# dcharatan/pixelsplat

Hardware: NVIDIA H100
Metric: rendered views/sec fwd+bwd @256x256, 3 gauss/px (higher is better)
Workload: dtype f32

## Files before the change

### include/pixelsplat_b200.h

```cpp
#ifndef PIXELSPLAT_B200_H
#define PIXELSPLAT_B200_H

#include <stddef.h>
#include <stdint.h>

#ifdef __cplusplus
extern "C" {
#endif

#if defined(__GNUC__)
#define PS_API __attribute__((visibility("default")))
#else
#define PS_API
#endif

#define PS_OK 0
#define PS_ERR_INVALID_ARGUMENT 1
#define PS_ERR_CUDA 2
#define PS_ERR_UNSUPPORTED 3

#define PS_TILE 16

#define PS_SH_M3 0
#define PS_SH_3M 1
// ... 21 lines not shown
#define PS_DEPTH_NONE 0
#define PS_DEPTH_Z 1
#define PS_DEPTH_DISPARITY 2
#define PS_DEPTH_RELATIVE_DISPARITY 3
#define PS_DEPTH_LOG 4

typedef struct ps_raster_inputs {
    const float *means;
    const float *cov;
    const float *opacities;
    const float *sh;
    const float *viewmatrix;
    const float *projmatrix;
    const float *campos;
    const float *tanfov;
    const float *background;
    const float *scene_scale;
    const float *near_far;
} ps_raster_inputs;

typedef struct ps_raster_state {
    void *geom;    size_t geom_bytes;
    void *binning; size_t binning_bytes;
    void *image;   size_t image_bytes;
} ps_raster_state;

typedef struct ps_raster_sizes {
    size_t geom_bytes, binning_bytes, image_bytes, backward_bytes;
} ps_raster_sizes;

typedef struct ps_raster_layout {
    size_t depth;
    size_t radii;
    size_t xy;
    size_t conic_opacity;
    size_t rgb;
    size_t rect;
    size_t clamped;
    size_t tile_count;
    size_t tile_start;
    size_t tile_cursor;
    size_t n_instances;
    size_t vis_pairs;
    size_t vis_any;
    size_t keys;
    size_t keys_alt;
    size_t final_T;
    size_t n_contrib;
    size_t cull;
    size_t color;
    size_t block_hits;
    size_t run_hits;
    size_t run_state;
    size_t depth_image;
    size_t run_depth;
} ps_raster_layout;

typedef struct ps_raster_camera_grads {
    float *d_viewmatrix;
    float *d_projmatrix;
    float *d_campos;
    float *d_tanfov;
    void *workspace;
    size_t workspace_bytes;
} ps_raster_camera_grads;

typedef struct ps_raster_grads {
    float *d_means;
    float *d_cov;
    float *d_opacities;
    float *d_sh;
    float *d_means2d;
    const ps_raster_camera_grads *camera;
} ps_raster_grads;

PS_API int ps_raster_camera_workspace_bytes(const ps_raster_desc *desc, size_t *out);

PS_API int ps_version(void);
PS_API const char *ps_last_error(void);

PS_API unsigned long long ps_launch_count(void);
PS_API void ps_timing_enable(int on);
PS_API int ps_timing_read(float *ms);

PS_API int ps_set_option(const char *name, int value);
PS_API int ps_get_option(const char *name, int *value);

PS_API int ps_raster_sizes_query(const ps_raster_desc *desc, ps_raster_sizes *out);
PS_API int ps_raster_layout_query(const ps_raster_desc *desc, ps_raster_layout *out);

PS_API int ps_camera_setup(int32_t n_views, const float *extrinsics, const float *intrinsics,
                           const float *near_plane, const float *far_plane, int32_t scale_invariant,
                           float *viewmatrix, float *projmatrix, float *campos, float *tanfov,
                           float *scene_scale, void *stream);

PS_API int ps_camera_setup_backward(int32_t n_views, const float *extrinsics, const float *intrinsics,
                                    const float *near_plane, const float *far_plane, int32_t scale_invariant,
                                    const float *d_viewmatrix, const float *d_projmatrix, const float *d_campos,
                                    const float *d_tanfov, float *d_extrinsics, float *d_intrinsics, void *stream);

PS_API int ps_raster_forward(const ps_raster_desc *desc, const ps_raster_inputs *in,
                      const ps_raster_state *state, float *out_color, int32_t *out_radii,
                      int64_t *n_instances_host, void *stream);

PS_API int ps_raster_backward(const ps_raster_desc *desc, const ps_raster_inputs *in,
                       const ps_raster_state *state, const float *d_color ,
                       void *scratch, size_t scratch_bytes, const ps_raster_grads *grads,
                       void *stream);


PS_API int ps_raster_backward_depth(const ps_raster_desc *desc, const ps_raster_inputs *in,
                                    const ps_raster_state *state, const float *d_color ,
                                    const float *loss_target, const float *grad_scale, const float *d_depth,
                                    void *scratch, size_t scratch_bytes, const ps_raster_grads *grads,
                                    void *stream);

#define PS_LOSS_SLOTS 64
typedef struct ps_raster_loss {
    const float *target;
    float *sums;
} ps_raster_loss;

PS_API int ps_raster_forward_loss(const ps_raster_desc *desc, const ps_raster_inputs *in,
                                  const ps_raster_state *state, const ps_raster_loss *loss,
                                  float *out_color , int32_t *out_radii,
                                  int64_t *n_instances_host, void *stream);
PS_API int ps_raster_backward_loss(const ps_raster_desc *desc, const ps_raster_inputs *in,
                                   const ps_raster_state *state, const float *target ,
                                   const float *grad_scale ,
                                   void *scratch, size_t scratch_bytes, const ps_raster_grads *grads,
                                   void *stream);

typedef struct ps_epipolar_desc {
    int32_t batch, views;
    int32_t grid_h, grid_w;
    int32_t samples;
    int32_t channels;
    int32_t heads;
    int32_t pe_dim;
} ps_epipolar_desc;

typedef struct ps_epipolar_inputs {
    const float *features;
    const float *segments;
    const uint8_t *valid;
    const float *rel_disparity;
    const float *q_feat;
    const float *q_pe;
    const float *bias;
} ps_epipolar_inputs;

PS_API int ps_epipolar_geometry(int32_t batch, int32_t views, int32_t grid_h, int32_t grid_w,
                                int32_t samples, const float *extrinsics ,
                                const float *intrinsics , const float *near_plane,
                                const float *far_plane , float *segments, uint8_t *valid,
                                float *rel_disparity, float *t_range, void *stream);

PS_API int ps_epipolar_attention_forward(const ps_epipolar_desc *desc, const ps_epipolar_inputs *in,
                                         float *z, float *e, float *mass, float *lse, void *stream);

PS_API int ps_epipolar_attention_backward(const ps_epipolar_desc *desc, const ps_epipolar_inputs *in,
                                          const float *lse, const float *dz, const float *de,
                                          const float *dmass, const float *d_row, float *dq_feat,
                                          float *dq_pe, float *dbias, float *dfeatures, void *stream);

PS_API int ps_epipolar_attention_backward_workspace_bytes(const ps_epipolar_desc *desc, size_t *out);
// ... 163 lines not shown
```

### pixelsplat_b200/_lib.py

```python
from __future__ import annotations

import ctypes
import os
from pathlib import Path

_PKG = Path(__file__).resolve().parent
LIB_PATH = Path(os.environ.get("PIXELSPLAT_B200_LIB", _PKG / "_C" / "libpixelsplat_b200.so"))

PS_OK = 0
PS_SH_M3, PS_SH_3M = 0, 1
PS_COV_TRIU6, PS_COV_3X3 = 0, 1
PS_SH_BASIS_3DGS, PS_SH_BASIS_E3NN = 0, 1
PS_ERR_UNSUPPORTED = 3
DEPTH_MODES = {None: 0, "depth": 1, "disparity": 2, "relative_disparity": 3, "log": 4}
TILE = 16

_ERR_NAMES = {1: "PS_ERR_INVALID_ARGUMENT", 2: "PS_ERR_CUDA", 3: "PS_ERR_UNSUPPORTED"}


class RasterDesc(ctypes.Structure):
    _fields_ = [
        ("n_scenes", ctypes.c_int32), ("views_per_scene", ctypes.c_int32),
        ("n_gaussians", ctypes.c_int32), ("sh_coeffs", ctypes.c_int32),
        ("sh_degree", ctypes.c_int32), ("sh_layout", ctypes.c_int32),
# ... 43 lines not shown
                ("sh_coeffs", ctypes.c_int32), ("image_h", ctypes.c_int32), ("image_w", ctypes.c_int32),
                ("scale_min", ctypes.c_float), ("scale_max", ctypes.c_float), ("eps", ctypes.c_float),
                ("reserved", ctypes.c_int32)]


class AdapterInputs(ctypes.Structure):
    _fields_ = [(n, ctypes.c_void_p) for n in (
        "extrinsics", "intrinsics", "sh_rotation", "sh_mask", "coordinates", "depths", "raw")]


class RasterLoss(ctypes.Structure):
    _fields_ = [("target", ctypes.c_void_p), ("sums", ctypes.c_void_p)]


LOSS_SLOTS = 64
LPIPS_MAX_LAYERS = 5


class LpipsLayer(ctypes.Structure):
    _fields_ = [("x0", ctypes.c_void_p), ("x1", ctypes.c_void_p), ("weight", ctypes.c_void_p),
                ("C", ctypes.c_int32), ("H", ctypes.c_int32), ("W", ctypes.c_int32)]


class LpipsDesc(ctypes.Structure):
    _fields_ = [("n_layers", ctypes.c_int32), ("N", ctypes.c_int32), ("layers", LpipsLayer * LPIPS_MAX_LAYERS),
                ("dropout_seed", ctypes.c_void_p)]


class LpipsGrads(ctypes.Structure):
    _fields_ = [("d_x0", ctypes.c_void_p * LPIPS_MAX_LAYERS), ("d_x1", ctypes.c_void_p * LPIPS_MAX_LAYERS)]


class ResampleDesc(ctypes.Structure):
    _fields_ = [(n, ctypes.c_int32) for n in ("n_images", "in_h", "in_w", "out_h", "out_w", "taps_h", "taps_v")] + \
        [(n, ctypes.c_void_p) for n in ("images", "flip", "bounds_h", "weights_h", "bounds_v", "weights_v")]


PS_EVAL_RENDER, PS_EVAL_FRAME = 0, 1
EVAL_MAX_IMAGES = 32


class EvalDesc(ctypes.Structure):
    _fields_ = [(n, ctypes.c_int32) for n in ("mode", "n_images", "height", "width")] + \
        [(n, ctypes.c_void_p) for n in ("render", "frame_in", "target", "frame_out", "planes", "sse")]


CLIP_ADAM_CHUNK = 4096
CLIP_ADAM_SEGMENT_FIELDS = ("param", "grad", "exp_avg", "exp_avg_sq", "count", "first_chunk")


class ClipAdamDesc(ctypes.Structure):
    _fields_ = [("n_segments", ctypes.c_int32), ("reserved", ctypes.c_int32), ("n_chunks", ctypes.c_int64),
                ("warm_up_steps", ctypes.c_int64)] + \
        [(n, ctypes.c_double) for n in ("lr", "beta1", "beta2", "eps", "max_norm")]


class ClipAdamState(ctypes.Structure):
    _fields_ = [("step", ctypes.c_void_p), ("grad_norm", ctypes.c_void_p)]


class RasterCameraGrads(ctypes.Structure):
    _fields_ = [(n, ctypes.c_void_p) for n in ("d_viewmatrix", "d_projmatrix", "d_campos", "d_tanfov", "workspace")] + \
        [("workspace_bytes", ctypes.c_size_t)]


class RasterGrads(ctypes.Structure):
    _fields_ = [(n, ctypes.c_void_p) for n in (
        "d_means", "d_cov", "d_opacities", "d_sh", "d_means2d")] + [("camera", ctypes.POINTER(RasterCameraGrads))]


EXPORTS = ("ps_version", "ps_last_error", "ps_raster_sizes_query", "ps_raster_layout_query",
           "ps_raster_forward", "ps_raster_backward", "ps_camera_setup", "ps_launch_count",
           "ps_timing_enable", "ps_timing_read", "ps_epipolar_geometry",
           "ps_epipolar_attention_forward", "ps_epipolar_attention_backward",
           "ps_self_attention_forward", "ps_gaussian_adapter_forward", "ps_gaussian_adapter_backward",
           "ps_sh_rotation_matrices", "ps_set_option", "ps_raster_forward_loss", "ps_raster_backward_loss",
           "ps_self_attention_forward_stats", "ps_self_attention_backward", "ps_get_option",
           "ps_raster_backward_depth", "ps_ssim_workspace_bytes", "ps_ssim_forward", "ps_ssim_backward",
           "ps_epipolar_attention_backward_workspace_bytes", "ps_epipolar_attention_backward_deterministic",
           "ps_raster_camera_workspace_bytes", "ps_camera_setup_backward", "ps_lpips_workspace_bytes",
           "ps_lpips_forward", "ps_lpips_backward", "ps_vit_attention_forward",
           "ps_vit_attention_backward_workspace_bytes", "ps_vit_attention_backward", "ps_image_resample",
           "ps_eval_images_workspace_bytes", "ps_eval_images", "ps_clip_adam_segment_chunks",
           "ps_clip_adam_workspace_bytes", "ps_clip_adam_step")


class NativeLibraryMissing(ImportError):
    pass


def _load() -> ctypes.CDLL:
    if not LIB_PATH.exists():
        raise NativeLibraryMissing(
            f"{LIB_PATH} not found: the sm_90a CUDA library is not built. Run "
            f"`make -C {_PKG / 'csrc'}` (or __graft_entry__.build()). There is no CPU fallback.")
    lib = ctypes.CDLL(str(LIB_PATH))
    lib.ps_version.restype = ctypes.c_int
    lib.ps_last_error.restype = ctypes.c_char_p
    P = ctypes.POINTER
    lib.ps_raster_sizes_query.argtypes = [P(RasterDesc), P(RasterSizes)]
    lib.ps_raster_layout_query.argtypes = [P(RasterDesc), P(RasterLayout)]
    lib.ps_raster_forward.argtypes = [P(RasterDesc), P(RasterInputs), P(RasterState), ctypes.c_void_p,
                                      ctypes.c_void_p, ctypes.c_void_p, ctypes.c_void_p]
    lib.ps_raster_backward.argtypes = [P(RasterDesc), P(RasterInputs), P(RasterState), ctypes.c_void_p,
                                       ctypes.c_void_p, ctypes.c_size_t, P(RasterGrads), ctypes.c_void_p]
    lib.ps_raster_forward_loss.argtypes = [P(RasterDesc), P(RasterInputs), P(RasterState), P(RasterLoss),
                                           ctypes.c_void_p, ctypes.c_void_p, ctypes.c_void_p, ctypes.c_void_p]
    lib.ps_raster_backward_loss.argtypes = [P(RasterDesc), P(RasterInputs), P(RasterState), ctypes.c_void_p,
                                            ctypes.c_void_p, ctypes.c_void_p, ctypes.c_size_t, P(RasterGrads),
                                            ctypes.c_void_p]
    lib.ps_raster_backward_depth.argtypes = [P(RasterDesc), P(RasterInputs), P(RasterState)] + [ctypes.c_void_p] * 5 + \
        [ctypes.c_size_t, P(RasterGrads), ctypes.c_void_p]
    lib.ps_raster_backward_depth.restype = ctypes.c_int
    lib.ps_raster_forward_loss.restype = ctypes.c_int
    lib.ps_raster_backward_loss.restype = ctypes.c_int
    lib.ps_camera_setup.argtypes = [ctypes.c_int32] + [ctypes.c_void_p] * 4 + [ctypes.c_int32] + \
        [ctypes.c_void_p] * 6
    lib.ps_camera_setup.restype = ctypes.c_int
    lib.ps_camera_setup_backward.argtypes = [ctypes.c_int32] + [ctypes.c_void_p] * 4 + [ctypes.c_int32] + \
        [ctypes.c_void_p] * 7
    lib.ps_camera_setup_backward.restype = ctypes.c_int
    lib.ps_raster_camera_workspace_bytes.argtypes = [P(RasterDesc), P(ctypes.c_size_t)]
    lib.ps_raster_camera_workspace_bytes.restype = ctypes.c_int
    lib.ps_launch_count.restype = ctypes.c_ulonglong
    lib.ps_timing_enable.argtypes = [ctypes.c_int]
    lib.ps_timing_enable.restype = None
    lib.ps_timing_read.argtypes = [ctypes.POINTER(ctypes.c_float)]
    lib.ps_timing_read.restype = ctypes.c_int
    lib.ps_epipolar_geometry.argtypes = [ctypes.c_int32] * 5 + [ctypes.c_void_p] * 9
    lib.ps_epipolar_geometry.restype = ctypes.c_int
    lib.ps_epipolar_attention_forward.argtypes = [P(EpipolarDesc), P(EpipolarInputs)] + [ctypes.c_void_p] * 5
    lib.ps_epipolar_attention_forward.restype = ctypes.c_int
    lib.ps_epipolar_attention_backward.argtypes = [P(EpipolarDesc), P(EpipolarInputs)] + [ctypes.c_void_p] * 10
    lib.ps_epipolar_attention_backward.restype = ctypes.c_int
    lib.ps_epipolar_attention_backward_workspace_bytes.argtypes = [P(EpipolarDesc), P(ctypes.c_size_t)]
    lib.ps_epipolar_attention_backward_workspace_bytes.restype = ctypes.c_int
    lib.ps_epipolar_attention_backward_deterministic.argtypes = [P(EpipolarDesc), P(EpipolarInputs)] + \
        [ctypes.c_void_p] * 10 + [ctypes.c_size_t, ctypes.c_void_p]
    lib.ps_epipolar_attention_backward_deterministic.restype = ctypes.c_int
    lib.ps_self_attention_forward.argtypes = [ctypes.c_int32] * 4 + [ctypes.c_void_p, ctypes.c_float, ctypes.c_void_p,
                                                                      ctypes.c_int32, ctypes.c_void_p]
    lib.ps_self_attention_forward.restype = ctypes.c_int
    lib.ps_self_attention_forward_stats.argtypes = [ctypes.c_int32] * 4 + [ctypes.c_void_p, ctypes.c_float,
                                                                            ctypes.c_void_p, ctypes.c_void_p, ctypes.c_void_p]
    lib.ps_self_attention_forward_stats.restype = ctypes.c_int
    lib.ps_self_attention_backward.argtypes = [ctypes.c_int32] * 4 + [ctypes.c_void_p] * 4 + [ctypes.c_float,
                                                                                             ctypes.c_void_p, ctypes.c_void_p]
    lib.ps_self_attention_backward.restype = ctypes.c_int
    lib.ps_gaussian_adapter_forward.argtypes = [P(AdapterDesc), P(AdapterInputs)] + [ctypes.c_void_p] * 6
    lib.ps_gaussian_adapter_forward.restype = ctypes.c_int
    lib.ps_gaussian_adapter_backward.argtypes = [P(AdapterDesc), P(AdapterInputs)] + [ctypes.c_void_p] * 9
    lib.ps_gaussian_adapter_backward.restype = ctypes.c_int
    lib.ps_sh_rotation_matrices.argtypes = [ctypes.c_int32] * 4 + [ctypes.c_void_p] * 5
    lib.ps_sh_rotation_matrices.restype = ctypes.c_int
    lib.ps_set_option.argtypes = [ctypes.c_char_p, ctypes.c_int]
    lib.ps_set_option.restype = ctypes.c_int
    lib.ps_get_option.argtypes = [ctypes.c_char_p, ctypes.POINTER(ctypes.c_int)]
    lib.ps_get_option.restype = ctypes.c_int
    lib.ps_ssim_workspace_bytes.argtypes = [ctypes.c_int32] * 3 + [P(ctypes.c_size_t)]
    lib.ps_ssim_workspace_bytes.restype = ctypes.c_int
    lib.ps_ssim_forward.argtypes = [ctypes.c_int32] * 3 + [ctypes.c_void_p] * 4 + [ctypes.c_size_t, ctypes.c_void_p]
    lib.ps_ssim_forward.restype = ctypes.c_int
    lib.ps_ssim_backward.argtypes = [ctypes.c_int32] * 3 + [ctypes.c_void_p] * 6 + [ctypes.c_size_t, ctypes.c_void_p]
    lib.ps_ssim_backward.restype = ctypes.c_int
    lib.ps_lpips_workspace_bytes.argtypes = [P(LpipsDesc), P(ctypes.c_size_t)]
    lib.ps_lpips_workspace_bytes.restype = ctypes.c_int
    lib.ps_lpips_forward.argtypes = [P(LpipsDesc), ctypes.c_void_p, ctypes.c_void_p, ctypes.c_size_t, ctypes.c_void_p]
    lib.ps_lpips_forward.restype = ctypes.c_int
    lib.ps_lpips_backward.argtypes = [P(LpipsDesc), ctypes.c_void_p, P(LpipsGrads), ctypes.c_void_p]
    lib.ps_lpips_backward.restype = ctypes.c_int
    lib.ps_vit_attention_forward.argtypes = [ctypes.c_int32] * 4 + [ctypes.c_void_p, ctypes.c_float] + \
        [ctypes.c_void_p] * 3
    lib.ps_vit_attention_forward.restype = ctypes.c_int
    lib.ps_vit_attention_backward_workspace_bytes.argtypes = [ctypes.c_int32] * 4 + [P(ctypes.c_size_t)]
    lib.ps_vit_attention_backward_workspace_bytes.restype = ctypes.c_int
    lib.ps_vit_attention_backward.argtypes = [ctypes.c_int32] * 4 + [ctypes.c_void_p] * 4 + \
        [ctypes.c_float, ctypes.c_void_p, ctypes.c_void_p, ctypes.c_size_t, ctypes.c_void_p]
    lib.ps_vit_attention_backward.restype = ctypes.c_int
    lib.ps_image_resample.argtypes = [P(ResampleDesc), ctypes.c_void_p, ctypes.c_void_p]
    lib.ps_image_resample.restype = ctypes.c_int
    lib.ps_eval_images_workspace_bytes.argtypes = [ctypes.c_int32] * 3 + [P(ctypes.c_size_t)]
    lib.ps_eval_images_workspace_bytes.restype = ctypes.c_int
    lib.ps_eval_images.argtypes = [P(EvalDesc), ctypes.c_void_p, ctypes.c_size_t, ctypes.c_void_p]
    lib.ps_eval_images.restype = ctypes.c_int
    lib.ps_clip_adam_segment_chunks.argtypes = [ctypes.c_void_p, ctypes.c_int64]
    lib.ps_clip_adam_segment_chunks.restype = ctypes.c_int64
    lib.ps_clip_adam_workspace_bytes.argtypes = [P(ClipAdamDesc), P(ctypes.c_size_t)]
    lib.ps_clip_adam_workspace_bytes.restype = ctypes.c_int
    lib.ps_clip_adam_step.argtypes = [P(ClipAdamDesc), ctypes.c_void_p, P(ClipAdamState), ctypes.c_void_p,
                                      ctypes.c_size_t, ctypes.c_void_p]
    lib.ps_clip_adam_step.restype = ctypes.c_int
    for f in ("ps_raster_sizes_query", "ps_raster_layout_query", "ps_raster_forward", "ps_raster_backward"):
        getattr(lib, f).restype = ctypes.c_int
    return lib


lib = _load()


class NativeError(RuntimeError):
    pass


def check(rc: int, what: str) -> None:
    if rc != PS_OK:
        msg = lib.ps_last_error().decode("utf-8", "replace")
        exc = ValueError if rc == 1 else NativeError
        raise exc(f"{what}: {_ERR_NAMES.get(rc, rc)}: {msg}")


def on_device(device, fn, *args) -> int:
# ... 40 lines not shown
```

### pixelsplat_b200/csrc/ps_common.cuh

```cuda
#pragma once
#include <cuda_runtime.h>
#include <stdint.h>

#include "../../include/pixelsplat_b200.h"

namespace ps {

constexpr int kTile = PS_TILE;
constexpr int kTilePixels = kTile * kTile;

struct Geom {
    float *depth;
    int32_t *radii;
    float2 *xy;
    float4 *conic_opacity;
    float4 *rgb;
    ushort4 *rect;
    uint8_t *clamped;
    uint32_t *tile_count;
    uint32_t *tile_start;
    uint32_t *tile_cursor;
    long long *n_instances;
    uint32_t *vis_pairs;
    float4 *cull;
// ... 51 lines not shown
__device__ __forceinline__ float depth_value(int mode, float vz, const float *scale, const float *near_far, int vid) {
    const float z = scale ? vz / scale[vid] : vz;
    if (mode == PS_DEPTH_DISPARITY) return 1.0f / z;
    if (mode == PS_DEPTH_RELATIVE_DISPARITY) {
        const float dn = 1.0f / (near_far[2 * vid] + kDepthEps), df = 1.0f / (near_far[2 * vid + 1] + kDepthEps);
        return 1.0f - (1.0f / (z + kDepthEps) - df) / (dn - df + kDepthEps);
    }
    if (mode == PS_DEPTH_LOG) return logf(fmaxf(fminf(z, near_far[2 * vid]), near_far[2 * vid + 1]));
    return z;
}

__device__ __forceinline__ float depth_value_grad(int mode, float vz, const float *scale, const float *near_far, int vid) {
    const float z = scale ? vz / scale[vid] : vz;
    if (mode == PS_DEPTH_DISPARITY) return -1.0f / (z * z);
    if (mode == PS_DEPTH_RELATIVE_DISPARITY) {
        const float dn = 1.0f / (near_far[2 * vid] + kDepthEps), df = 1.0f / (near_far[2 * vid + 1] + kDepthEps);
        const float iz = 1.0f / (z + kDepthEps);
        return iz * iz / (dn - df + kDepthEps);
    }
    if (mode == PS_DEPTH_LOG) {
        const float nr = near_far[2 * vid], fr = near_far[2 * vid + 1];
        const float m = fminf(z, nr);
        const float gm = z < nr ? 1.0f : (z == nr ? 0.5f : 0.0f);
        const float gr = m > fr ? 1.0f : (m == fr ? 0.5f : 0.0f);
        return gm * gr / fmaxf(m, fr);
    }
    return 1.0f;
}

__device__ __forceinline__ float2 cull_extent(float a, float c, float o) {
    if (!(a > 0.0f) || !(c > 0.0f) || !(o <= 3.0e38f)) return make_float2(3.0e38f, 3.0e38f);
    if (!(o * 255.0f >= 1.0f - 1e-3f)) return make_float2(-3.0e38f, -3.0e38f);
    const float tau2 = 2.0f * (__logf(fmaxf(o * 255.0f, 1.0f)) + 0.01f);
    return make_float2(sqrtf(tau2 * a) * 1.001f + 0.01f, sqrtf(tau2 * c) * 1.001f + 0.01f);
}

constexpr uint32_t kLivePosLimit = 1u << 24;

__device__ __forceinline__ uint32_t tile_block_mask(const float4 &cr, int x0, int y0) {
    const float xl = cr.x - cr.z, xh = cr.x + cr.z, yl = cr.y - cr.w, yh = cr.y + cr.w;
    uint32_t xm = 0, m = 0;
#pragma unroll
    for (int bx = 0; bx < 2; ++bx)
        xm |= ((xh >= (float)(x0 + 8 * bx)) && (xl <= (float)(x0 + 8 * bx + 7))) ? 1u << bx : 0u;
#pragma unroll
    for (int by = 0; by < 4; ++by)
        m |= ((yh >= (float)(y0 + 4 * by)) && (yl <= (float)(y0 + 4 * by + 3))) ? xm << (2 * by) : 0u;
    return m;
}

void set_error(const char *fmt, ...);

enum Mark { kMarkFwdStart = 0, kMarkPreprocess, kMarkScatter, kMarkSort, kMarkCompositeFwd,
            kMarkBwdStart, kMarkBwdZero, kMarkCompositeBwd, kMarkPreprocessBwd, kNumMarks };
void mark(int id, cudaStream_t st);
void count_launch();

bool first_use_on_device(unsigned long long &mask);

#define PS_CUDA_CHECK(expr)                                                              \
    do {                                                                                 \
        cudaError_t _e = (expr);                                                         \
        if (_e != cudaSuccess) {                                                         \
            ps::set_error("%s failed: %s (%s:%d)", #expr, cudaGetErrorString(_e), __FILE__, __LINE__); \
            return PS_ERR_CUDA;                                                          \
        }                                                                                \
    } while (0)

#define PS_LAUNCH_CHECK(name)                                                            \
    do {                                                                                 \
        cudaError_t _e = cudaGetLastError();                                             \
        if (_e != cudaSuccess) {                                                         \
            ps::set_error("launch of %s failed: %s", name, cudaGetErrorString(_e));      \
            return PS_ERR_CUDA;                                                          \
        }                                                                                \
        ps::count_launch();                                                              \
    } while (0)

int launch_preprocess(const Dims &d, const Inputs &in, const Geom &g, cudaStream_t st);
int launch_sh_color(const Dims &d, const Inputs &in, const Geom &g, cudaStream_t st);
int launch_binning(const Dims &d, const Geom &g, unsigned long long *keys,
                   unsigned long long *keys_alt, int sort_impl, int segment_hint, cudaEvent_t scanned,
                   cudaStream_t st);
int launch_composite_forward(const Dims &d, const Inputs &in, const Geom &g,
                             const unsigned long long *keys, const uint2 *live, const ImageState &img,
                             float *out_color, const LossEpilogue &loss, const HitLists &hl, float *loss_partials,
                             cudaStream_t st);
int launch_composite_backward(const Dims &d, const Inputs &in, const Geom &g,
                              const unsigned long long *keys, const uint2 *live, const ImageState &img,
                              const float *d_color, const float *d_depth, const ViewGrads &vg,
                              const ViewGrads *records, const LossEpilogue &loss, const HitLists &hl,
                              cudaStream_t st);
int launch_composite_forward_v1(const Dims &d, const Inputs &in, const Geom &g,
                                const unsigned long long *keys, const ImageState &img,
                                float *out_color, cudaStream_t st);
int launch_composite_backward_v1(const Dims &d, const Inputs &in, const Geom &g,
                                 const unsigned long long *keys, const ImageState &img,
                                 const float *d_color, const ViewGrads &vg, cudaStream_t st);
int composite_impl();
int set_composite_option(int which, int value);
int get_composite_option(int which);
int composite_segments(long long tasks);
bool composite_hit_lists(long long capacity);
int launch_preprocess_backward(const Dims &d, const Inputs &in, const Geom &g, const ViewGrads &vg,
                               const ps_raster_grads &grads, cudaStream_t st);
int launch_clear_pair_grads(const Dims &d, const Geom &g, const ViewGrads &vg, cudaStream_t st);

}
```

### pixelsplat_b200/csrc/raster_api.cu

```cuda
#include <cstdarg>
#include <atomic>
#include <cstdio>
#include <cstring>
#include <mutex>

#include "ps_common.cuh"

namespace ps {

static thread_local char g_error[512] = "";

void set_error(const char *fmt, ...) {
    va_list ap;
    va_start(ap, fmt);
    vsnprintf(g_error, sizeof(g_error), fmt, ap);
    va_end(ap);
}

static bool g_timing = false;
static cudaEvent_t g_events[kNumMarks];
static bool g_events_ready = false;
static std::atomic<unsigned long long> g_launches{0};

void count_launch() { g_launches.fetch_add(1, std::memory_order_relaxed); }
// ... 183 lines not shown
}

static ImageState make_image(const Layout &L, void *image) {
    char *b = static_cast<char *>(image);
    ImageState im;
    im.final_T = reinterpret_cast<float *>(b + L.off.final_T);
    im.n_contrib = reinterpret_cast<uint32_t *>(b + L.off.n_contrib);
    im.color = reinterpret_cast<float *>(b + L.off.color);
    im.run_state = reinterpret_cast<float4 *>(b + L.off.run_state);
    im.depth_image = L.off.depth_image ? reinterpret_cast<float *>(b + L.off.depth_image) : nullptr;
    im.run_depth = L.off.run_depth ? reinterpret_cast<float *>(b + L.off.run_depth) : nullptr;
    return im;
}

static int check_common(const ps_raster_desc *desc, const ps_raster_inputs *in, const ps_raster_state *state,
                        const Layout &L, bool backward) {
    const size_t image_bytes = backward && L.det ? L.loss_partials : L.sizes.image_bytes;
    if (!in || !state) { set_error("inputs/state is NULL"); return PS_ERR_INVALID_ARGUMENT; }
    if (!in->means || !in->cov || !in->opacities || !in->sh || !in->viewmatrix || !in->projmatrix ||
        !in->campos || !in->tanfov || !in->background) {
        set_error("a required input pointer is NULL");
        return PS_ERR_INVALID_ARGUMENT;
    }
    if (!state->geom || !state->binning || !state->image) { set_error("a state buffer is NULL"); return PS_ERR_INVALID_ARGUMENT; }
    if (state->geom_bytes < L.sizes.geom_bytes || state->binning_bytes < L.sizes.binning_bytes ||
        state->image_bytes < image_bytes) {
        set_error("state buffers too small: need geom %zu binning %zu image %zu, got %zu %zu %zu",
                  L.sizes.geom_bytes, L.sizes.binning_bytes, image_bytes, state->geom_bytes,
                  state->binning_bytes, state->image_bytes);
        return PS_ERR_INVALID_ARGUMENT;
    }
    if (((uintptr_t)state->geom | (uintptr_t)state->binning | (uintptr_t)state->image) & 15) {
        set_error("state buffers must be 16-byte aligned");
        return PS_ERR_INVALID_ARGUMENT;
    }
    if ((desc->depth_mode == PS_DEPTH_RELATIVE_DISPARITY || desc->depth_mode == PS_DEPTH_LOG) && !in->near_far) {
        set_error("depth_mode %d needs ps_raster_inputs.near_far", desc->depth_mode);
        return PS_ERR_INVALID_ARGUMENT;
    }
    if (desc->depth_mode && composite_impl() == 1) {
        set_error("the legacy compositor (composite_impl = 1) has no depth channel");
        return PS_ERR_UNSUPPORTED;
    }
    if (L.det && composite_impl() == 1) {
        set_error("the legacy compositor (composite_impl = 1) has no fixed-order (deterministic) form");
        return PS_ERR_UNSUPPORTED;
    }
    return PS_OK;
}

static Inputs make_inputs(const ps_raster_inputs *in) {
    Inputs r;
    r.means = in->means; r.cov = in->cov; r.opac = in->opacities; r.sh = in->sh;
    r.view = in->viewmatrix; r.proj = in->projmatrix; r.campos = in->campos; r.tanfov = in->tanfov;
    r.bg = in->background; r.scale = in->scene_scale; r.near_far = in->near_far;
    return r;
}

}

using namespace ps;

extern "C" {

PS_API int ps_version(void) { return 100; }

PS_API const char *ps_last_error(void) { return g_error; }

PS_API unsigned long long ps_launch_count(void) { return g_launches.load(std::memory_order_relaxed); }

PS_API void ps_timing_enable(int on) { g_timing = on != 0; }

PS_API int ps_timing_read(float *ms) {
    if (!g_timing || !g_events_ready) { set_error("timing is not enabled"); return PS_ERR_INVALID_ARGUMENT; }
    static const int pairs[7][2] = {{kMarkFwdStart, kMarkPreprocess}, {kMarkPreprocess, kMarkScatter},
                                    {kMarkScatter, kMarkSort}, {kMarkSort, kMarkCompositeFwd},
                                    {kMarkBwdStart, kMarkBwdZero}, {kMarkBwdZero, kMarkCompositeBwd},
                                    {kMarkCompositeBwd, kMarkPreprocessBwd}};
    PS_CUDA_CHECK(cudaEventSynchronize(g_events[kMarkPreprocessBwd]));
    for (int i = 0; i < 7; ++i) PS_CUDA_CHECK(cudaEventElapsedTime(&ms[i], g_events[pairs[i][0]], g_events[pairs[i][1]]));
    return PS_OK;
}

PS_API int ps_set_option(const char *name, int value) {
    if (!name) { set_error("ps_set_option: name is NULL"); return PS_ERR_INVALID_ARGUMENT; }
    int rc = PS_ERR_INVALID_ARGUMENT;
    if (!strcmp(name, "composite_impl")) rc = set_composite_option(0, value);
    else if (!strcmp(name, "composite_segments")) rc = set_composite_option(1, value);
    else if (!strcmp(name, "composite_hit_lists")) rc = set_composite_option(2, value);
    else if (!strcmp(name, "deterministic") && (value == 0 || value == 1)) { g_deterministic = value; rc = PS_OK; }
    if (rc) set_error("ps_set_option: unknown option or bad value: %s = %d", name, value);
    return rc;
}

PS_API int ps_get_option(const char *name, int *value) {
    if (!name || !value) { set_error("ps_get_option: name / value is NULL"); return PS_ERR_INVALID_ARGUMENT; }
    int which = -1;
    if (!strcmp(name, "composite_impl")) which = 0;
    else if (!strcmp(name, "composite_segments")) which = 1;
    else if (!strcmp(name, "composite_hit_lists")) which = 2;
    else if (!strcmp(name, "deterministic")) { *value = g_deterministic; return PS_OK; }
    if (which < 0) { set_error("ps_get_option: unknown option %s", name); return PS_ERR_INVALID_ARGUMENT; }
    *value = get_composite_option(which);
    return PS_OK;
}

PS_API int ps_raster_sizes_query(const ps_raster_desc *desc, ps_raster_sizes *out) {
    int rc = validate(desc);
    if (rc) return rc;
    if (!out) { set_error("out is NULL"); return PS_ERR_INVALID_ARGUMENT; }
    *out = make_layout(desc).sizes;
    return PS_OK;
}

PS_API int ps_raster_layout_query(const ps_raster_desc *desc, ps_raster_layout *out) {
    int rc = validate(desc);
    if (rc) return rc;
    if (!out) { set_error("out is NULL"); return PS_ERR_INVALID_ARGUMENT; }
    *out = make_layout(desc).off;
    return PS_OK;
}

PS_API int ps_raster_camera_workspace_bytes(const ps_raster_desc *desc, size_t *out) {
    int rc = validate(desc);
    if (rc) return rc;
    if (!out) { set_error("out is NULL"); return PS_ERR_INVALID_ARGUMENT; }
    *out = camera_workspace_bytes(desc);
    return PS_OK;
}

}

static int raster_forward_impl(const ps_raster_desc *desc, const ps_raster_inputs *in, const ps_raster_state *state,
                               float *out_color, int32_t *out_radii, int64_t *n_instances_host,
                               const ps_raster_loss *loss, void *stream) {
    int rc = validate(desc);
    if (rc) return rc;
    const Layout L = make_layout(desc);
    rc = check_common(desc, in, state, L, false);
    if (rc) return rc;
    LossEpilogue le{nullptr, nullptr, nullptr};
    if (loss) {
        if (!loss->target || !loss->sums) { set_error("ps_raster_loss: target / sums is NULL"); return PS_ERR_INVALID_ARGUMENT; }
        le.target = loss->target; le.sums = loss->sums;
    } else if (!out_color) {
        set_error("out_color is NULL");
        return PS_ERR_INVALID_ARGUMENT;
    }
    cudaStream_t st = static_cast<cudaStream_t>(stream);
    const Dims d = make_dims(desc);
    const Inputs I = make_inputs(in);
    const Geom g = make_geom(L, state->geom);
    unsigned long long *keys = reinterpret_cast<unsigned long long *>(static_cast<char *>(state->binning) + L.off.keys);
    unsigned long long *keys_alt = reinterpret_cast<unsigned long long *>(static_cast<char *>(state->binning) + L.off.keys_alt);
    const ImageState img = make_image(L, state->image);

    SideCtx *sc = nullptr;
    if ((rc = side_ready(sc))) return rc;
    std::lock_guard<std::mutex> enqueue_lock(sc->enqueue);
    mark(kMarkFwdStart, st);
    if ((rc = launch_preprocess(d, I, g, st))) return rc;
    mark(kMarkPreprocess, st);
    PS_CUDA_CHECK(cudaEventRecord(sc->fork, st));
    PS_CUDA_CHECK(cudaStreamWaitEvent(sc->side, sc->fork, 0));
    if ((rc = launch_sh_color(d, I, g, sc->side))) return rc;
    PS_CUDA_CHECK(cudaEventRecord(sc->join, sc->side));
// ... 152 lines not shown
```

### pixelsplat_b200/csrc/raster_binning.cu

```cuda
#include <cub/device/device_segmented_radix_sort.cuh>

#include "ps_common.cuh"

namespace ps {

constexpr int kScanThreads = 1024;

__global__ void __launch_bounds__(kScanThreads)
k_tile_scan(int n, const uint32_t *__restrict__ count, uint32_t *__restrict__ start,
            uint32_t *__restrict__ cursor, long long *__restrict__ n_instances) {
    __shared__ uint32_t warp_sums[32];
    __shared__ unsigned long long carry_s;
    const int tid = threadIdx.x, lane = tid & 31, warp = tid >> 5;
    if (tid == 0) carry_s = 0;
    __syncthreads();
    uint32_t cmax = 0;
    for (int base = 0; base < n; base += kScanThreads) {
        const int i = base + tid;
        const uint32_t c = i < n ? count[i] : 0u;
        cmax = max(cmax, c);
        uint32_t x = c;
#pragma unroll
        for (int o = 1; o < 32; o <<= 1) {
            const uint32_t y = __shfl_up_sync(0xffffffffu, x, o);
            if (lane >= o) x += y;
        }
        if (lane == 31) warp_sums[warp] = x;
        __syncthreads();
        if (warp == 0) {
            uint32_t w = warp_sums[lane];
#pragma unroll
            for (int o = 1; o < 32; o <<= 1) {
                const uint32_t y = __shfl_up_sync(0xffffffffu, w, o);
                if (lane >= o) w += y;
            }
            warp_sums[lane] = w;
        }
        __syncthreads();
        const unsigned long long carry = carry_s;
        const uint32_t warp_off = warp ? warp_sums[warp - 1] : 0u;
        const unsigned long long excl = carry + warp_off + (x - c);
        if (i < n) {
            const uint32_t e = excl > 0xffffffffull ? 0xffffffffu : (uint32_t)excl;
            start[i] = e;
            cursor[i] = e;
        }
        __syncthreads();
        if (tid == kScanThreads - 1) carry_s = carry + warp_sums[31];
        __syncthreads();
    }
    if (tid == 0) *n_instances = (long long)carry_s;
    cmax = __reduce_max_sync(0xffffffffu, cmax);
    if (lane == 0 && cmax) atomicMax(reinterpret_cast<unsigned long long *>(n_instances + 1), (unsigned long long)cmax);
}

constexpr int kScatterThreads = 256;
constexpr int kScatterMaxSmemTiles = 8192;

__global__ void __launch_bounds__(kScatterThreads)
k_scatter(Dims d, Geom geo, unsigned long long *__restrict__ keys, int use_smem) {
    extern __shared__ uint32_t s_scatter[];
    if (*geo.n_instances > d.capacity) return;
    const int vid = blockIdx.y;
    const int g = blockIdx.x * kScatterThreads + threadIdx.x;
    uint32_t *cnt = s_scatter, *base = s_scatter + d.tiles;
    uint32_t *cur = geo.tile_cursor + (size_t)vid * d.tiles;
    const size_t vg = (size_t)vid * d.P + g;
    const bool vis = g < d.P && geo.radii[vg] > 0;
    ushort4 r = make_ushort4(0, 0, 0, 0);
    unsigned long long key = 0;
    if (vis) {
        r = geo.rect[vg];
        key = ((unsigned long long)__float_as_uint(geo.depth[vg]) << 32) | (uint32_t)g;
    }
    if (!use_smem) {
        for (int ty = r.y; ty < r.w; ++ty)
            for (int tx = r.x; tx < r.z; ++tx) keys[atomicAdd(&cur[ty * d.gx + tx], 1u)] = key;
        return;
    }
    for (int i = threadIdx.x; i < d.tiles; i += kScatterThreads) cnt[i] = 0;
    __syncthreads();
    for (int ty = r.y; ty < r.w; ++ty)
        for (int tx = r.x; tx < r.z; ++tx) atomicAdd(&cnt[ty * d.gx + tx], 1u);
    __syncthreads();
    for (int i = threadIdx.x; i < d.tiles; i += kScatterThreads) {
        const uint32_t c = cnt[i];
        if (c) { base[i] = atomicAdd(&cur[i], c); cnt[i] = 0; }
    }
    __syncthreads();
    for (int ty = r.y; ty < r.w; ++ty)
        for (int tx = r.x; tx < r.z; ++tx) {
            const int t = ty * d.gx + tx;
            keys[base[t] + atomicAdd(&cnt[t], 1u)] = key;
        }
}

template <int THREADS>
__device__ void bitonic_sort_smem(unsigned long long *s_keys, int n_pad) {
    constexpr int kWarps = THREADS / 32;
    const int lane = threadIdx.x & 31, warp = threadIdx.x >> 5;
    const int chunk = max(n_pad / kWarps, 2);
    const int warps_used = n_pad / chunk;
    const int half = n_pad >> 1;
    for (int k = 2; k <= n_pad; k <<= 1) {
        int j = k >> 1;
        const bool had_global = j >= chunk;
        for (; j >= chunk; j >>= 1) {
            for (int t = threadIdx.x; t < half; t += THREADS) {
                const int i = 2 * t - (t & (j - 1));
                const int p = i + j;
                const unsigned long long a = s_keys[i], b = s_keys[p];
                const bool up = (i & k) == 0;
                if ((a > b) == up) { s_keys[i] = b; s_keys[p] = a; }
            }
            __syncthreads();
        }
        if (warp < warps_used) {
            const int base = warp * chunk;
            for (; j > 0; j >>= 1) {
                for (int t = lane; t < (chunk >> 1); t += 32) {
                    const int i = base + 2 * t - (t & (j - 1));
                    const int p = i + j;
                    const unsigned long long a = s_keys[i], b = s_keys[p];
                    const bool up = (i & k) == 0;
                    if ((a > b) == up) { s_keys[i] = b; s_keys[p] = a; }
                }
                __syncwarp();
            }
        }
        if (had_global || 2 * k > chunk) __syncthreads();
    }
}

constexpr int kSortThreads = 512;
constexpr int kSortWarps = kSortThreads / 32;

constexpr int kLiveItems = 4;
static_assert(kLiveItems * kSortWarps == 64, "write_live_list scans the (item, warp) counts two per lane");

struct SortSmem {
    uint32_t cnt[kSortWarps * 256];
    uint32_t misc[64];
    uint32_t live[kLiveItems * kSortWarps];
};

__device__ unsigned long long *radix8_passes(unsigned long long *a, unsigned long long *b, int n, SortSmem &sm,
                                             int key_shift, uint32_t sub, int num_passes) {
    const int tid = threadIdx.x, lane = tid & 31, warp = tid >> 5;
    const int lo = (int)(((long long)n * warp) / kSortWarps);
    const int hi = (int)(((long long)n * (warp + 1)) / kSortWarps);
    uint32_t *cnt = sm.cnt, *misc = sm.misc;
    for (int p = 0; p < num_passes; ++p) {
        const int shift = 8 * p;
        auto digit = [&](unsigned long long k) -> uint32_t {
            return ((((uint32_t)(k >> key_shift)) - sub) >> shift) & 255u;
        };
        for (int i = tid; i < kSortWarps * 256; i += kSortThreads) cnt[i] = 0;
        if (tid == 0) misc[0] = 0;
        __syncthreads();
        for (int i = lo + lane; i < hi; i += 32) atomicAdd(&cnt[warp * 256 + digit(a[i])], 1u);
        __syncthreads();
        uint32_t total = 0, incl = 0;
        if (tid < 256) {
            uint32_t c[kSortWarps];
#pragma unroll
            for (int w = 0; w < kSortWarps; ++w) c[w] = cnt[w * 256 + tid];
#pragma unroll
            for (int w = 0; w < kSortWarps; ++w) { const uint32_t t = c[w]; c[w] = total; total += t; }
            if (total == (uint32_t)n) misc[0] = 1;
            incl = total;
#pragma unroll
            for (int o = 1; o < 32; o <<= 1) {
                const uint32_t y = __shfl_up_sync(0xffffffffu, incl, o);
                if (lane >= o) incl += y;
            }
            if (lane == 31) misc[8 + warp] = incl;
#pragma unroll
            for (int w = 0; w < kSortWarps; ++w) cnt[w * 256 + tid] = c[w];
        }
        __syncthreads();
        if (misc[0]) { __syncthreads(); continue; }
        if (tid < 256) {
            uint32_t off = incl - total;
            for (int w = 0; w < warp; ++w) off += misc[8 + w];
#pragma unroll
            for (int w = 0; w < kSortWarps; ++w) cnt[w * 256 + tid] += off;
        }
        __syncthreads();
        for (int base = lo; base < hi; base += 32) {
            const int i = base + lane;
            const bool valid = i < hi;
            const unsigned long long key = valid ? a[i] : 0ull;
            const uint32_t dg = valid ? digit(key) : (256u + (uint32_t)lane);
            const uint32_t peers = __match_any_sync(0xffffffffu, dg);
            const int leader = __ffs(peers) - 1;
            const int rank = __popc(peers & ((1u << lane) - 1u));
            uint32_t off = 0;
            if (valid && lane == leader) {
                off = cnt[warp * 256 + dg];
                cnt[warp * 256 + dg] = off + (uint32_t)__popc(peers);
            }
            off = __shfl_sync(0xffffffffu, off, leader);
            if (valid) b[off + rank] = key;
            __syncwarp();
        }
        __syncthreads();
        unsigned long long *t = a; a = b; b = t;
    }
    return a;
}

static size_t sort_smem_bytes(int cap) { return sizeof(SortSmem) + sizeof(unsigned long long) * 2 * (size_t)cap; }

__device__ void write_live_list(const Dims &d, const Geom &geo, const unsigned long long *sorted, int n, int seg,
                                uint2 *__restrict__ live, SortSmem &sm) {
    const int tid = threadIdx.x, lane = tid & 31, warp = tid >> 5;
    const int vid = seg / d.tiles, tile = seg - vid * d.tiles;
    const int x0 = (tile % d.gx) * kTile, y0 = (tile / d.gx) * kTile;
    const float4 *__restrict__ cull = geo.cull + (size_t)vid * d.P;
    const bool keep_all = (uint32_t)n > kLivePosLimit;
    uint32_t carry = 0;
    for (int base = 0; base < n; base += kSortThreads * kLiveItems) {
        uint32_t g[kLiveItems];
        float4 cr[kLiveItems];
#pragma unroll
        for (int k = 0; k < kLiveItems; ++k) {
            const int i = base + k * kSortThreads + tid;
            g[k] = i < n ? (uint32_t)sorted[i] : 0u;
            cr[k] = i < n ? cull[g[k]] : make_float4(0.0f, 0.0f, -3.0e38f, -3.0e38f);
        }
        uint32_t mask[kLiveItems], ballot[kLiveItems];
#pragma unroll
        for (int k = 0; k < kLiveItems; ++k) {
            const int i = base + k * kSortThreads + tid;
            mask[k] = i < n ? tile_block_mask(cr[k], x0, y0) : 0u;
            ballot[k] = __ballot_sync(0xffffffffu, i < n && (mask[k] != 0u || keep_all));
            if (lane == 0) sm.live[k * kSortWarps + warp] = (uint32_t)__popc(ballot[k]);
        }
        __syncthreads();
        const uint32_t c0 = sm.live[lane], c1 = sm.live[32 + lane];
        uint32_t e0 = c0, e1 = c1;
#pragma unroll
        for (int o = 1; o < 32; o <<= 1) {
            const uint32_t y0 = __shfl_up_sync(0xffffffffu, e0, o), y1 = __shfl_up_sync(0xffffffffu, e1, o);
            if (lane >= o) { e0 += y0; e1 += y1; }
        }
        const uint32_t half = __shfl_sync(0xffffffffu, e0, 31);
        const uint32_t total = half + __shfl_sync(0xffffffffu, e1, 31);
        e0 -= c0;
        e1 += half - c1;
        uint32_t off[kLiveItems];
        off[0] = carry + __shfl_sync(0xffffffffu, e0, warp);
        off[1] = carry + __shfl_sync(0xffffffffu, e0, 16 + warp);
        off[2] = carry + __shfl_sync(0xffffffffu, e1, warp);
        off[3] = carry + __shfl_sync(0xffffffffu, e1, 16 + warp);
        carry += total;
#pragma unroll
        for (int k = 0; k < kLiveItems; ++k) {
            const int i = base + k * kSortThreads + tid;
            if ((ballot[k] >> lane) & 1u)
                live[off[k] + (uint32_t)__popc(ballot[k] & ((1u << lane) - 1u))] =
                    make_uint2(((uint32_t)i << 8) | mask[k], g[k]);
        }
        __syncthreads();
    }
    if (tid == 0) geo.tile_cursor[seg] = carry;
}

__global__ void __launch_bounds__(kSortThreads)
k_tile_sort(Dims d, Geom geo, unsigned long long *__restrict__ keys, unsigned long long *__restrict__ keys_alt,
            int cap, int id_bits) {
    extern __shared__ __align__(16) unsigned char s_sort[];
    if (*geo.n_instances > d.capacity) return;
    const int seg = blockIdx.x;
    const int n = (int)geo.tile_count[seg];
    const uint32_t s0 = geo.tile_start[seg];
    SortSmem &sm = *reinterpret_cast<SortSmem *>(s_sort);
    uint2 *live = reinterpret_cast<uint2 *>(keys_alt + s0);
    if (n < 2) { write_live_list(d, geo, keys + s0, n, seg, live, sm); return; }
    const int tid = threadIdx.x, lane = tid & 31;
    if (n > cap) {
        unsigned long long *r = radix8_passes(keys + s0, keys_alt + s0, n, sm, 0, 0u, (id_bits + 7) / 8);
        unsigned long long *o = (r == keys + s0) ? keys_alt + s0 : keys + s0;
        r = radix8_passes(r, o, n, sm, 32, 0u, 4);
        if (r != keys + s0)
            for (int i = tid; i < n; i += kSortThreads) keys[s0 + i] = r[i];
        __syncthreads();
        write_live_list(d, geo, keys + s0, n, seg, live, sm);
        return;
    }
    unsigned long long *A = reinterpret_cast<unsigned long long *>(s_sort + sizeof(SortSmem));
    unsigned long long *B = A + cap;
    if (tid == 0) { sm.misc[1] = 0xffffffffu; sm.misc[2] = 0u; sm.misc[3] = 0u; }
    __syncthreads();
    uint32_t dlo = 0xffffffffu, dhi = 0u;
    for (int i = tid; i < n; i += kSortThreads) {
        const unsigned long long k = keys[s0 + i];
        A[i] = k;
        const uint32_t dpt = (uint32_t)(k >> 32);
        dlo = min(dlo, dpt); dhi = max(dhi, dpt);
    }
    dlo = __reduce_min_sync(0xffffffffu, dlo);
    dhi = __reduce_max_sync(0xffffffffu, dhi);
    if (lane == 0) { atomicMin(&sm.misc[1], dlo); atomicMax(&sm.misc[2], dhi); }
    __syncthreads();
    const uint32_t dmin = sm.misc[1], range = sm.misc[2] - dmin;
    const int bits = range ? 32 - __clz(range) : 0;
    __syncthreads();
    A = radix8_passes(A, B, n, sm, 32, dmin, (bits + 7) / 8);
    for (int i = tid; i < n; i += kSortThreads) {
        const uint32_t dpt = (uint32_t)(A[i] >> 32);
        const bool starts = (i == 0 || (uint32_t)(A[i - 1] >> 32) != dpt) && (i + 1 < n) &&
                            (uint32_t)(A[i + 1] >> 32) == dpt;
        if (starts) {
            int e = i + 2;
            while (e < n && (uint32_t)(A[e] >> 32) == dpt) ++e;
            if (e - i > 64) {
                sm.misc[3] = 1u;
            } else {
                for (int x = i + 1; x < e; ++x) {
                    const unsigned long long v = A[x];
                    int y = x - 1;
                    while (y >= i && A[y] > v) { A[y + 1] = A[y]; --y; }
                    A[y + 1] = v;
                }
            }
        }
    }
    __syncthreads();
    if (sm.misc[3]) {
        int n_pad = 2;
        while (n_pad < n) n_pad <<= 1;
        for (int i = n + tid; i < n_pad; i += kSortThreads) A[i] = ~0ull;
        __syncthreads();
        bitonic_sort_smem<kSortThreads>(A, n_pad);
    }
    for (int i = tid; i < n; i += kSortThreads) keys[s0 + i] = A[i];
    write_live_list(d, geo, A, n, seg, live, sm);
}

__global__ void __launch_bounds__(kSortThreads)
k_live_lists(Dims d, Geom geo, const unsigned long long *__restrict__ keys, unsigned long long *__restrict__ keys_alt) {
    __shared__ SortSmem sm;
    if (*geo.n_instances > d.capacity) return;
    const int seg = blockIdx.x;
    const uint32_t s0 = geo.tile_start[seg];
    write_live_list(d, geo, keys + s0, (int)geo.tile_count[seg], seg, reinterpret_cast<uint2 *>(keys_alt + s0), sm);
}

int launch_binning(const Dims &d, const Geom &g, unsigned long long *keys,
                   unsigned long long *keys_alt, int sort_impl, int segment_hint, cudaEvent_t scanned,
                   cudaStream_t st) {
    const int n_seg = d.S * d.V * d.tiles;
    k_tile_scan<<<1, kScanThreads, 0, st>>>(n_seg, g.tile_count, g.tile_start, g.tile_cursor, g.n_instances);
    PS_LAUNCH_CHECK("k_tile_scan");
    if (scanned) PS_CUDA_CHECK(cudaEventRecord(scanned, st));
    const int use_smem = d.tiles <= kScatterMaxSmemTiles;
    static unsigned long long scatter_attr_devices = 0;
    if (first_use_on_device(scatter_attr_devices)) {
        PS_CUDA_CHECK(cudaFuncSetAttribute(k_scatter, cudaFuncAttributeMaxDynamicSharedMemorySize,
                                           (int)(2 * sizeof(uint32_t) * kScatterMaxSmemTiles)));
    }
    dim3 sgrid((d.P + kScatterThreads - 1) / kScatterThreads, d.S * d.V);
    k_scatter<<<sgrid, kScatterThreads, use_smem ? 2 * sizeof(uint32_t) * d.tiles : 0, st>>>(d, g, keys, use_smem);
    PS_LAUNCH_CHECK("k_scatter");
    mark(kMarkScatter, st);

    int id_bits = 1;
    while ((1ll << id_bits) < d.P) ++id_bits;

    if (sort_impl == 1) {
        size_t temp = 0;
        cub::DoubleBuffer<unsigned long long> db(keys, keys_alt);
        PS_CUDA_CHECK(cub::DeviceSegmentedRadixSort::SortKeys(nullptr, temp, db, (int)d.capacity, n_seg,
                                                              g.tile_start, g.tile_cursor, 0, 64, st));
        void *tmp = nullptr;
        PS_CUDA_CHECK(cudaMallocAsync(&tmp, temp, st));
        PS_CUDA_CHECK(cub::DeviceSegmentedRadixSort::SortKeys(tmp, temp, db, (int)d.capacity, n_seg,
                                                              g.tile_start, g.tile_cursor, 0, 64, st));
        if (db.Current() != keys)
            PS_CUDA_CHECK(cudaMemcpyAsync(keys, db.Current(), sizeof(unsigned long long) * (size_t)d.capacity,
                                          cudaMemcpyDeviceToDevice, st));
        PS_CUDA_CHECK(cudaFreeAsync(tmp, st));
        k_live_lists<<<n_seg, kSortThreads, 0, st>>>(d, g, keys, keys_alt);
        PS_LAUNCH_CHECK("k_live_lists");
        return PS_OK;
    }

    int cap = 2048;
    if (segment_hint > 0) {
        const long long want = (long long)segment_hint + segment_hint / 4;
        while (cap < want && cap < 8192) cap <<= 1;
    }
    static unsigned long long battr_devices = 0;
    if (first_use_on_device(battr_devices)) {
        PS_CUDA_CHECK(cudaFuncSetAttribute(k_tile_sort, cudaFuncAttributeMaxDynamicSharedMemorySize,
                                           (int)sort_smem_bytes(8192)));
    }
    k_tile_sort<<<n_seg, kSortThreads, sort_smem_bytes(cap), st>>>(d, g, keys, keys_alt, cap, id_bits);
    PS_LAUNCH_CHECK("k_tile_sort");
    return PS_OK;
}

}
```

Baseline: 3103.

## Use 9-bit radix digits and finer shared-memory capacity steps in tile sort

The per-tile radix sort now uses up to 9-bit digits with one digit per thread (512 threads) and an adaptive digit width, so fewer passes are needed. The match_any peer detection is replaced by a per-bit ballot loop. Sort capacity is rounded to 512-element steps instead of powers of two, which cuts dynamic shared memory and may allow more CTAs per SM. A query API for capacity and occupancy is added. The trade-off is larger per-warp count arrays and more ballots per key.

```diff
diff --git a/include/pixelsplat_b200.h b/include/pixelsplat_b200.h
--- a/include/pixelsplat_b200.h
+++ b/include/pixelsplat_b200.h
@@ -127,6 +127,7 @@
 PS_API unsigned long long ps_launch_count(void);
 PS_API void ps_timing_enable(int on);
 PS_API int ps_timing_read(float *ms);
+PS_API int ps_tile_sort_config(int32_t segment_hint, int32_t *cap, int32_t *ctas_per_sm);
 
 PS_API int ps_set_option(const char *name, int value);
 PS_API int ps_get_option(const char *name, int *value);
diff --git a/pixelsplat_b200/_lib.py b/pixelsplat_b200/_lib.py
--- a/pixelsplat_b200/_lib.py
+++ b/pixelsplat_b200/_lib.py
@@ -149,7 +149,7 @@
            "ps_lpips_forward", "ps_lpips_backward", "ps_vit_attention_forward",
            "ps_vit_attention_backward_workspace_bytes", "ps_vit_attention_backward", "ps_image_resample",
            "ps_eval_images_workspace_bytes", "ps_eval_images", "ps_clip_adam_segment_chunks",
-           "ps_clip_adam_workspace_bytes", "ps_clip_adam_step")
+           "ps_clip_adam_workspace_bytes", "ps_clip_adam_step", "ps_tile_sort_config")
 
 
 class NativeLibraryMissing(ImportError):
@@ -194,6 +194,8 @@
     lib.ps_timing_enable.restype = None
     lib.ps_timing_read.argtypes = [ctypes.POINTER(ctypes.c_float)]
     lib.ps_timing_read.restype = ctypes.c_int
+    lib.ps_tile_sort_config.argtypes = [ctypes.c_int32, P(ctypes.c_int32), P(ctypes.c_int32)]
+    lib.ps_tile_sort_config.restype = ctypes.c_int
     lib.ps_epipolar_geometry.argtypes = [ctypes.c_int32] * 5 + [ctypes.c_void_p] * 9
     lib.ps_epipolar_geometry.restype = ctypes.c_int
     lib.ps_epipolar_attention_forward.argtypes = [P(EpipolarDesc), P(EpipolarInputs)] + [ctypes.c_void_p] * 5
diff --git a/pixelsplat_b200/csrc/ps_common.cuh b/pixelsplat_b200/csrc/ps_common.cuh
--- a/pixelsplat_b200/csrc/ps_common.cuh
+++ b/pixelsplat_b200/csrc/ps_common.cuh
@@ -157,6 +157,7 @@
 int launch_binning(const Dims &d, const Geom &g, unsigned long long *keys,
                    unsigned long long *keys_alt, int sort_impl, int segment_hint, cudaEvent_t scanned,
                    cudaStream_t st);
+int tile_sort_config(int segment_hint, int *cap, int *ctas_per_sm);
 int launch_composite_forward(const Dims &d, const Inputs &in, const Geom &g,
                              const unsigned long long *keys, const uint2 *live, const ImageState &img,
                              float *out_color, const LossEpilogue &loss, const HitLists &hl, float *loss_partials,
diff --git a/pixelsplat_b200/csrc/raster_api.cu b/pixelsplat_b200/csrc/raster_api.cu
--- a/pixelsplat_b200/csrc/raster_api.cu
+++ b/pixelsplat_b200/csrc/raster_api.cu
@@ -289,6 +289,16 @@
     return PS_OK;
 }
 
+PS_API int ps_tile_sort_config(int32_t segment_hint, int32_t *cap, int32_t *ctas_per_sm) {
+    if (!cap || !ctas_per_sm) { set_error("ps_tile_sort_config: cap / ctas_per_sm is NULL"); return PS_ERR_INVALID_ARGUMENT; }
+    int c = 0, n = 0;
+    const int rc = tile_sort_config(segment_hint, &c, &n);
+    if (rc) return rc;
+    *cap = c;
+    *ctas_per_sm = n;
+    return PS_OK;
+}
+
 PS_API int ps_set_option(const char *name, int value) {
     if (!name) { set_error("ps_set_option: name is NULL"); return PS_ERR_INVALID_ARGUMENT; }
     int rc = PS_ERR_INVALID_ARGUMENT;
diff --git a/pixelsplat_b200/csrc/raster_binning.cu b/pixelsplat_b200/csrc/raster_binning.cu
--- a/pixelsplat_b200/csrc/raster_binning.cu
+++ b/pixelsplat_b200/csrc/raster_binning.cu
@@ -1,3 +1,5 @@
+#include <algorithm>
+
 #include <cub/device/device_segmented_radix_sort.cuh>
 
 #include "ps_common.cuh"
@@ -138,70 +140,79 @@
 constexpr int kLiveItems = 4;
 static_assert(kLiveItems * kSortWarps == 64, "write_live_list scans the (item, warp) counts two per lane");
 
+constexpr int kDigitBits = 9;
+constexpr int kDigits = 1 << kDigitBits;
+static_assert(kDigits == kSortThreads, "the column scan gives each thread one digit");
+
 struct SortSmem {
-    uint32_t cnt[kSortWarps * 256];
+    uint32_t cnt[kSortWarps * kDigits];
     uint32_t misc[64];
     uint32_t live[kLiveItems * kSortWarps];
 };
 
-__device__ unsigned long long *radix8_passes(unsigned long long *a, unsigned long long *b, int n, SortSmem &sm,
-                                             int key_shift, uint32_t sub, int num_passes) {
+__device__ unsigned long long *radix_passes(unsigned long long *a, unsigned long long *b, int n, SortSmem &sm,
+                                            int key_shift, uint32_t sub, int bits) {
     const int tid = threadIdx.x, lane = tid & 31, warp = tid >> 5;
     const int lo = (int)(((long long)n * warp) / kSortWarps);
     const int hi = (int)(((long long)n * (warp + 1)) / kSortWarps);
+    const int num_passes = (bits + kDigitBits - 1) / kDigitBits;
+    const int width = num_passes ? (bits + num_passes - 1) / num_passes : 0;
+    const uint32_t mask = (1u << width) - 1u;
     uint32_t *cnt = sm.cnt, *misc = sm.misc;
     for (int p = 0; p < num_passes; ++p) {
-        const int shift = 8 * p;
+        const int shift = width * p;
         auto digit = [&](unsigned long long k) -> uint32_t {
-            return ((((uint32_t)(k >> key_shift)) - sub) >> shift) & 255u;
+            return ((((uint32_t)(k >> key_shift)) - sub) >> shift) & mask;
         };
-        for (int i = tid; i < kSortWarps * 256; i += kSortThreads) cnt[i] = 0;
+        for (int i = tid; i < kSortWarps * kDigits; i += kSortThreads) cnt[i] = 0;
         if (tid == 0) misc[0] = 0;
         __syncthreads();
-        for (int i = lo + lane; i < hi; i += 32) atomicAdd(&cnt[warp * 256 + digit(a[i])], 1u);
-        __syncthreads();
-        uint32_t total = 0, incl = 0;
-        if (tid < 256) {
-            uint32_t c[kSortWarps];
-#pragma unroll
-            for (int w = 0; w < kSortWarps; ++w) c[w] = cnt[w * 256 + tid];
-#pragma unroll
-            for (int w = 0; w < kSortWarps; ++w) { const uint32_t t = c[w]; c[w] = total; total += t; }
-            if (total == (uint32_t)n) misc[0] = 1;
-            incl = total;
-#pragma unroll
-            for (int o = 1; o < 32; o <<= 1) {
-                const uint32_t y = __shfl_up_sync(0xffffffffu, incl, o);
-                if (lane >= o) incl += y;
-            }
-            if (lane == 31) misc[8 + warp] = incl;
-#pragma unroll
-            for (int w = 0; w < kSortWarps; ++w) cnt[w * 256 + tid] = c[w];
-        }
+        for (int i = lo + lane; i < hi; i += 32) atomicAdd(&cnt[warp * kDigits + digit(a[i])], 1u);
+        __syncthreads();
+        uint32_t c[kSortWarps];
+        uint32_t total = 0;
+#pragma unroll
+        for (int w = 0; w < kSortWarps; ++w) c[w] = cnt[w * kDigits + tid];
+#pragma unroll
+        for (int w = 0; w < kSortWarps; ++w) { const uint32_t t = c[w]; c[w] = total; total += t; }
+        if (total == (uint32_t)n) misc[0] = 1;
+        uint32_t incl = total;
+#pragma unroll
+        for (int o = 1; o < 32; o <<= 1) {
+            const uint32_t y = __shfl_up_sync(0xffffffffu, incl, o);
+            if (lane >= o) incl += y;
+        }
+        if (lane == 31) misc[8 + warp] = incl;
         __syncthreads();
         if (misc[0]) { __syncthreads(); continue; }
-        if (tid < 256) {
-            uint32_t off = incl - total;
-            for (int w = 0; w < warp; ++w) off += misc[8 + w];
-#pragma unroll
-            for (int w = 0; w < kSortWarps; ++w) cnt[w * 256 + tid] += off;
-        }
+        uint32_t off = incl - total;
+        for (int w = 0; w < warp; ++w) off += misc[8 + w];
+#pragma unroll
+        for (int w = 0; w < kSortWarps; ++w) cnt[w * kDigits + tid] = c[w] + off;
         __syncthreads();
         for (int base = lo; base < hi; base += 32) {
             const int i = base + lane;
             const bool valid = i < hi;
             const unsigned long long key = valid ? a[i] : 0ull;
-            const uint32_t dg = valid ? digit(key) : (256u + (uint32_t)lane);
-            const uint32_t peers = __match_any_sync(0xffffffffu, dg);
-            const int leader = __ffs(peers) - 1;
+            const uint32_t dg = valid ? digit(key) : 0u;
+            uint32_t peers = __ballot_sync(0xffffffffu, valid);
+#pragma unroll
+            for (int bit = 0; bit < kDigitBits; ++bit) {
+                if (bit < width) {
+                    const bool set = (dg >> bit) & 1u;
+                    const uint32_t ones = __ballot_sync(0xffffffffu, set);
+                    peers &= set ? ones : ~ones;
+                }
+            }
+            const int leader = valid ? __ffs(peers) - 1 : lane;
             const int rank = __popc(peers & ((1u << lane) - 1u));
-            uint32_t off = 0;
+            uint32_t o = 0;
             if (valid && lane == leader) {
-                off = cnt[warp * 256 + dg];
-                cnt[warp * 256 + dg] = off + (uint32_t)__popc(peers);
-            }
-            off = __shfl_sync(0xffffffffu, off, leader);
-            if (valid) b[off + rank] = key;
+                o = cnt[warp * kDigits + dg];
+                cnt[warp * kDigits + dg] = o + (uint32_t)__popc(peers);
+            }
+            o = __shfl_sync(0xffffffffu, o, leader);
+            if (valid) b[o + rank] = key;
             __syncwarp();
         }
         __syncthreads();
@@ -280,17 +291,17 @@
     if (n < 2) { write_live_list(d, geo, keys + s0, n, seg, live, sm); return; }
     const int tid = threadIdx.x, lane = tid & 31;
     if (n > cap) {
-        unsigned long long *r = radix8_passes(keys + s0, keys_alt + s0, n, sm, 0, 0u, (id_bits + 7) / 8);
+        unsigned long long *r = radix_passes(keys + s0, keys_alt + s0, n, sm, 0, 0u, id_bits);
         unsigned long long *o = (r == keys + s0) ? keys_alt + s0 : keys + s0;
-        r = radix8_passes(r, o, n, sm, 32, 0u, 4);
+        r = radix_passes(r, o, n, sm, 32, 0u, 32);
         if (r != keys + s0)
             for (int i = tid; i < n; i += kSortThreads) keys[s0 + i] = r[i];
         __syncthreads();
         write_live_list(d, geo, keys + s0, n, seg, live, sm);
         return;
     }
-    unsigned long long *A = reinterpret_cast<unsigned long long *>(s_sort + sizeof(SortSmem));
-    unsigned long long *B = A + cap;
+    unsigned long long *const S = reinterpret_cast<unsigned long long *>(s_sort + sizeof(SortSmem));
+    unsigned long long *A = S, *B = S + cap;
     if (tid == 0) { sm.misc[1] = 0xffffffffu; sm.misc[2] = 0u; sm.misc[3] = 0u; }
     __syncthreads();
     uint32_t dlo = 0xffffffffu, dhi = 0u;
@@ -307,7 +318,7 @@
     const uint32_t dmin = sm.misc[1], range = sm.misc[2] - dmin;
     const int bits = range ? 32 - __clz(range) : 0;
     __syncthreads();
-    A = radix8_passes(A, B, n, sm, 32, dmin, (bits + 7) / 8);
+    A = radix_passes(A, B, n, sm, 32, dmin, bits);
     for (int i = tid; i < n; i += kSortThreads) {
         const uint32_t dpt = (uint32_t)(A[i] >> 32);
         const bool starts = (i == 0 || (uint32_t)(A[i - 1] >> 32) != dpt) && (i + 1 < n) &&
@@ -331,6 +342,11 @@
     if (sm.misc[3]) {
         int n_pad = 2;
         while (n_pad < n) n_pad <<= 1;
+        if (A != S) {
+            for (int i = tid; i < n; i += kSortThreads) S[i] = A[i];
+            A = S;
+            __syncthreads();
+        }
         for (int i = n + tid; i < n_pad; i += kSortThreads) A[i] = ~0ull;
         __syncthreads();
         bitonic_sort_smem<kSortThreads>(A, n_pad);
@@ -346,6 +362,23 @@
     const int seg = blockIdx.x;
     const uint32_t s0 = geo.tile_start[seg];
     write_live_list(d, geo, keys + s0, (int)geo.tile_count[seg], seg, reinterpret_cast<uint2 *>(keys_alt + s0), sm);
+}
+
+constexpr int kCapStep = 512;
+
+static int sort_capacity(int segment_hint) {
+    if (segment_hint <= 0) return 2048;
+    const long long want = (long long)segment_hint + segment_hint / 4;
+    return (int)std::min(8192ll, std::max((long long)kCapStep, (want + kCapStep - 1) / kCapStep * kCapStep));
+}
+
+static int sort_attributes() {
+    static unsigned long long battr_devices = 0;
+    if (first_use_on_device(battr_devices)) {
+        PS_CUDA_CHECK(cudaFuncSetAttribute(k_tile_sort, cudaFuncAttributeMaxDynamicSharedMemorySize,
+                                           (int)sort_smem_bytes(8192)));
+    }
+    return PS_OK;
 }
 
 int launch_binning(const Dims &d, const Geom &g, unsigned long long *keys,
@@ -387,19 +420,19 @@
         return PS_OK;
     }
 
-    int cap = 2048;
-    if (segment_hint > 0) {
-        const long long want = (long long)segment_hint + segment_hint / 4;
-        while (cap < want && cap < 8192) cap <<= 1;
-    }
-    static unsigned long long battr_devices = 0;
-    if (first_use_on_device(battr_devices)) {
-        PS_CUDA_CHECK(cudaFuncSetAttribute(k_tile_sort, cudaFuncAttributeMaxDynamicSharedMemorySize,
-                                           (int)sort_smem_bytes(8192)));
-    }
+    const int cap = sort_capacity(segment_hint);
+    if (int rc = sort_attributes()) return rc;
     k_tile_sort<<<n_seg, kSortThreads, sort_smem_bytes(cap), st>>>(d, g, keys, keys_alt, cap, id_bits);
     PS_LAUNCH_CHECK("k_tile_sort");
     return PS_OK;
 }
 
-}
+int tile_sort_config(int segment_hint, int *cap, int *ctas_per_sm) {
+    *cap = sort_capacity(segment_hint);
+    if (int rc = sort_attributes()) return rc;
+    PS_CUDA_CHECK(cudaOccupancyMaxActiveBlocksPerMultiprocessor(ctas_per_sm, k_tile_sort, kSortThreads,
+                                                                sort_smem_bytes(*cap)));
+    return PS_OK;
+}
+
+}
```

After: 3142, median of 6. 1.3% higher.
